# A2R-Lab/indy7-mpc

Measured on AMD Instinct MI355X. Metric: SQP-MPC solves/sec (Indy7 6-DOF, N=32), higher is better.
Workload: dtype f64

## Files before the change

### indy7_mpc_amd/csrc/i7m_admm.h

```cpp
#pragma once

#include "i7m_kernels.h"

namespace i7m {

struct AdmmCfg {
  double rho0, sigma, alpha, eps_abs, eps_rel, adapt_tol;
  int max_iter, check, scaling, gap, adapt_interval, pad;
};

struct AdmmArgs {
  SolveParams P;
  AdmmCfg A;
  const double* lin;
  const double* cost;
  const double* qpd;
  const double* xu;
  const double* xs;
  const int* active;
  double* sol;
  double *sx, *sz, *sy, *sq, *srho;
  double *Pq, *Pd, *I, *qs, *ls, *D, *E, *Dt, *Et, *R, *w;
  double* cs;
  int* iters;
  int* status;
  int sqp_iter;
  int b0;
  int ablate;
  const double* abase;
  long abytes;
};

constexpr int ADMM_FSTRIDE = 19;
constexpr int ADMM_SCALE_WPE = 2;
constexpr int ADMM_FACTOR_WPE = 2;
constexpr int ADM_REC = 300, REC_J = 180;
__device__ __forceinline__ int adm_lw(int i) { return i < 16 ? 2 * ((i + 2) / 2) : 18; }
__device__ __forceinline__ int adm_lrow(int i) {
  const int h = i >> 1;
  return i < 16 ? 2 * h * (h + 1) + (i & 1) * (2 * h + 2) : 144 + 18 * (i - 16);
}
__device__ __forceinline__ int adm_lrec(int i, int j) { return adm_lrow(i) + j; }
constexpr unsigned A5_OOB = 0x7ff00000u;
__device__ __forceinline__ __amdgpu_buffer_rsrc_t a4_rsrc(const void* base, long bytes) {
  const unsigned long long u = (unsigned long long)base;
  const unsigned lo = __builtin_amdgcn_readfirstlane((unsigned)u), hi = __builtin_amdgcn_readfirstlane((unsigned)(u >> 32));
  const int nb = __builtin_amdgcn_readfirstlane((int)bytes);
  return __builtin_amdgcn_make_buffer_rsrc((void*)(((unsigned long long)hi << 32) | lo), (short)0, nb, 0x00020000);
}
__device__ __forceinline__ void adm_stage_J(double* sJ, const double* Jc, int l) {
  for (int e = l; e < 216; e += 64) {
    const int i = e / 18, j = e - 18 * i;
    double v;
    if (i < 6) v = j == i ? Jc[i] : (j == 6 + i ? Jc[6 + i] : 0.0);
    else v = Jc[12 + 18 * (i - 6) + j];
    sJ[e] = v;
  }
}

// ... 112 lines not shown
    xPx += xe * px;
    qx += qe * xe;
  }
  pr = adm_max<W>(pr); zn = adm_max<W>(zn); an = adm_max<W>(an); pri = adm_max<W>(pri); pn = adm_max<W>(pn);
  dr = adm_max<W>(dr); qn = adm_max<W>(qn); atn = adm_max<W>(atn); pxn = adm_max<W>(pxn);
  dua = adm_max<W>(dua); dn = adm_max<W>(dn);
  xPx = adm_sum<W>(xPx); qx = adm_sum<W>(qx); sc = adm_sum<W>(sc);
  const double cinv = 1.0 / c;
  {
    const double p = pri / (pn + 1e-30), d = dua / (dn + 1e-30);
    double rn = rho * sqrt(p / (d + 1e-30));
    *rho_est = fmin(fmax(rn, 1e-6), 1e6);
  }
  dr *= cinv;
  const double ea = es * a.A.eps_abs, er = es * a.A.eps_rel;
  if (!(pr < ea + er * fmax(zn, an))) return false;
  if (!(dr < ea + er * cinv * fmax(qn, fmax(atn, pxn)))) return false;
  if (a.A.gap) {
    xPx *= cinv; qx *= cinv; sc *= cinv;
    const double gp = xPx + qx + sc;
    if (!(fabs(gp) < ea + er * fmax(fabs(xPx), fmax(fabs(qx), fabs(sc))))) return false;
  }
  return true;
}

__device__ __forceinline__ double adm_pq(const double* w, int i, int j) { return w[6] * (w[i] * w[j]); }
template <int CT>
__device__ __forceinline__ double adm_scale(const AdmmArgs& a, int b, int N, int T, int m, const double* LIN,
                                            const double* CO, const double* QD, const double* X, double* qold,
                                            double* Pq, double* Pd, double* Jb, double* Ib, double* qs, double* ls,
                                            double* D, double* E, double* sD, double* sE, double* sDt, double* sRM, int l) {
  constexpr int RT = 2 * CT / 3;
  const double dt = a.P.dt;
  double qv[CT], etv[RT], dtv[CT <= 9 ? CT : 1];
#pragma unroll
  for (int t = 0; t < CT; ++t) {
    const int e = l + 64 * t;
    qv[t] = 0.0;
    if (e < T) {
      sD[e] = 1.0;
      qv[t] = qold[e];
    }
  }
#pragma unroll
  for (int t = 0; t < RT; ++t)
    if (l + 64 * t < m) sE[l + 64 * t] = 1.0;
  wave_sync_fence();
  double c = 1.0;
  auto pcol = [&](const double* Cp, int k, int j, double dj) {
    const double* w = Cp + COST_STRIDE * k;
    const int jq = j < 6 ? j : 0;
    double mq = 0.0;
#pragma unroll
    for (int i = 0; i < 6; ++i) mq = fmax(mq, fabs(adm_pq(w, i, jq)) * (sD[18 * k + i] * dj) * c);
    const double pd = j < 12 ? w[7] : w[8];
    return j < 6 ? mq : fabs(pd) * (dj * dj) * c;
  };
  constexpr bool REG = CT <= 9;
  const int ks = l >> 1, hs = l & 1;
  const bool sv = REG && ks < N - 1;
  double av[REG ? 3 : 1][REG ? 18 : 1];
  if constexpr (REG) {
    const double* L = LIN + LIN_STRIDE * (sv ? ks : 0);
#pragma unroll
    for (int r = 0; r < 3; ++r)
#pragma unroll
      for (int j = 0; j < 18; ++j) {
// ... 34 lines not shown
      for (int j = 0; j < 18; ++j) {
        const long long u = __double_as_longlong(cm[j]);
        const int lo = __builtin_amdgcn_update_dpp(0, (int)u, 0xB1, 0xf, 0xf, true);
        const int hi = __builtin_amdgcn_update_dpp(0, (int)(u >> 32), 0xB1, 0xf, 0xf, true);
        cm[j] = fmax(cm[j], __longlong_as_double(((long long)hi << 32) | (unsigned int)lo));
      }
      if (sv) {
#pragma unroll
        for (int j = 0; j < 9; ++j) sDt[18 * kq + 9 * hs + j] = hs ? cm[9 + j] : cm[j];
      }
      wave_sync_fence();
    }
    AS_STAMP(1);
#pragma unroll 3
    for (int t = 0; t < CT; ++t) {
      const int e = min(lp + 64 * t, T - 1), k = e / 18, j = e - 18 * k;
      const double dj = sD[e];
      double mx = pcol(Cp, k, j, dj);
      const double ei = sE[12 * k + (j < 12 ? j : 0)] * dj;
      if (j < 12) mx = fmax(mx, ei);
      const int kk = k < N - 1 ? k : N - 2;
      const double* L = Lp + LIN_STRIDE * kk;
      const double* Eb = sE + 12 * (kk + 1);
      const int jb = j < 6 ? j : (j < 12 ? 30 + j : 60 + j);
      const double eid = Eb[j < 6 ? j : (j < 12 ? j - 6 : 0)] * (j < 6 ? 1.0 : dt) * dj;
      double mj = j < 12 ? eid : 0.0;
      if constexpr (REG) {
        mj = fmax(mj, sDt[e]);
      } else {
#pragma unroll
        for (int r = 0; r < 6; ++r) mj = fmax(mj, Eb[6 + r] * fabs(L[jb + 6 * r]) * dj);
      }
      if (k < N - 1) mx = fmax(mx, mj);
      if constexpr (REG) dtv[t] = 1.0 / sqrt(adm_limit(mx));
      else sDt[lp + 64 * t] = 1.0 / sqrt(adm_limit(mx));
    }
    AS_STAMP(2);
#pragma unroll
    for (int t = 0; t < RT; ++t) {
      const int r = min(lp + 64 * t, m - 1), blk = r / 12, i = r - 12 * blk;
      const double er = sE[r];
      double mx = er * sD[18 * blk + i];
      const int kk = blk > 0 ? blk - 1 : 0;
      const double* Db = sD + 18 * kk;
      const int i6 = i < 6 ? i : i - 6;
      const double mi = fmax(er * 1.0 * Db[i6], er * dt * Db[6 + i6]);
      double ml = 0.0;
      if constexpr (REG) {
        ml = sRM[r];
      } else {
        const double* L = Lp + LIN_STRIDE * kk;
#pragma unroll
        for (int j = 0; j < 18; ++j) {
          const int jb = j < 6 ? j : (j < 12 ? 30 + j : 60 + j);
          ml = fmax(ml, er * fabs(L[jb + 6 * i6]) * Db[j]);
        }
      }
      const double mj = i < 6 ? mi : ml;
      if (blk > 0) mx = fmax(mx, mj);
      etv[t] = 1.0 / sqrt(adm_limit(mx));
    }
    AS_STAMP(3);
    wave_sync_fence();
#pragma unroll
    for (int t = 0; t < CT; ++t) {
      const int e = lp + 64 * t;
      double dtt;
      if constexpr (CT <= 9) dtt = dtv[t];
      else dtt = sDt[e];
      if (e < T) sD[e] = sD[e] * dtt;
      qv[t] = dtt * qv[t];
    }
#pragma unroll
    for (int t = 0; t < RT; ++t)
      if (lp + 64 * t < m) sE[lp + 64 * t] = sE[lp + 64 * t] * etv[t];
    wave_sync_fence();
    AS_STAMP(4);
    double sm = 0.0, qm = 0.0;
#pragma unroll
    for (int t = 0; t < CT; ++t) {
      const int e = lp + 64 * t, ec = min(e, T - 1), k = ec / 18, j = ec - 18 * k;
      const double mx = pcol(Cp, k, j, sD[ec]);
      if (e < T) {
        sm += mx;
        qm = fmax(qm, fabs(qv[t]));
      }
    }
    sm = adm_wave_sum(sm);
    qm = adm_limit(adm_wave_max(qm));
    const double ct = 1.0 / adm_limit(fmax(sm / T, qm));
#pragma unroll
    for (int t = 0; t < CT; ++t) qv[t] = qv[t] * ct;
    c = c * ct;
    AS_STAMP(5);
  }
#undef AS_STAMP
#ifdef I7M_DIAG
  if (ss_on && l == 0) tl_write_stamps(ss_t, 6, a.ablate, 3);
#endif
  for (int e = l; e < T; e += 64) D[e] = sD[e];
  for (int r = l; r < m; r += 64) E[r] = sE[r];
#pragma unroll 4
// ... 175 lines not shown
        sL[18 * i + l] = v;
        if (l < adm_lw(i)) Rb[ADM_REC * k + adm_lrec(i, l)] = v;
      }
    }
    wave_sync();
    AF_STAMP(5);
    if (k < N - 1) {
#pragma unroll
      for (int t = 0; t < 4; ++t) {
        const int e = l + 64 * t;
        if (e < 216) {
          const int i = e / 18, j = e - 18 * i;
          const double acc = adm_dot2<18>(0.0, sJ + 18 * i, 1, sL + 18 * j, 1);
          const double cv = re * G[186 + i] * acc;
          sCp[FS * i + j] = cv;
        }
      }
    }
    wave_sync_fence();
    AF_STAMP(6);
  }
#undef AF_STAMP
#ifdef I7M_DIAG
  if (fs_on && l0 == 0) tl_write_stamps(fs_t, 7, a.ablate, 2);
#endif
}

template <int PH, int CT>
__device__ __forceinline__ void admm_body(const AdmmArgs& a) {
  const int b = a.b0 + blockIdx.x;
  const SolveParams& P = a.P;
  if (b >= P.B || (a.active && !a.active[b])) return;
  const int l = threadIdx.x, N = P.N, T = P.T, m = 12 * N;
  constexpr bool FAC = (PH & 8) != 0;
  __shared__ double sB[(PH & 1) ? 64 * CT : 756], sS[FAC ? 18 * ADMM_FSTRIDE : 1], sCp[FAC ? 12 * ADMM_FSTRIDE : 1];
  __shared__ double sD[(PH & 1) ? 64 * CT : 1], sE[(PH & 1) ? 64 * (2 * CT / 3) : 1], sRM[(PH & 1) ? 64 * (2 * CT / 3) : 1],
      sCO[(PH & 1) ? (64 * CT / 18 + 1) * COST_STRIDE : 1], sStg[FAC ? 2 * AF_STG : 1];
  double* sL = sB;
  double* sJ = sB + 540;
  const double* LIN = a.lin + (long)b * (N - 1) * LIN_STRIDE;
  const double* CO = a.cost + (long)b * N * COST_STRIDE;
  const double* QD = a.qpd + (long)b * (N - 1) * QPD_STRIDE;
  const double* X = a.xu + (long)b * T;
  double* qold = a.sq + (long)b * T;
  double* Pq = a.Pq + (long)b * N * 36;
  double* Pd = a.Pd + (long)b * T;
  double* Rb = a.R + (long)b * N * ADM_REC;
  double* Jb = Rb + REC_J;
  double* Ib = a.I + (long)b * m;
  double* qs = a.qs + (long)b * T;
  double* ls = a.ls + (long)b * m;
  double* D = a.D + (long)b * T;
  double* E = a.E + (long)b * m;
  if constexpr (PH & 1) {
    for (int e = l; e < N * COST_STRIDE; e += 64) sCO[e] = CO[e];
    const double c = adm_scale<CT>(a, b, N, T, m, LIN, sCO, QD, X, qold, Pq, Pd, Jb, Ib, qs, ls, D, E, sD, sE, sB, sRM, l);
    if (l == 0) a.cs[b] = c;
  }
  if constexpr (PH & 8) {
    adm_factor(a, N, a.srho[b], Pq, Pd, Ib, Rb, sS, sJ, sL, sCp, sStg, l);
  }
}

template <int CT>
__global__ void __launch_bounds__(64) __attribute__((amdgpu_waves_per_eu(ADMM_SCALE_WPE, ADMM_SCALE_WPE)))
k_admm_scale(AdmmArgs a) {
  admm_body<1, CT>(a);
}
__global__ void __launch_bounds__(64) __attribute__((amdgpu_waves_per_eu(ADMM_FACTOR_WPE, ADMM_FACTOR_WPE)))
k_admm_factor(AdmmArgs a) {
  admm_body<8, 1>(a);
}

}
```

### indy7_mpc_amd/csrc/i7m_admm_prep_tu.hip

```cpp
#include <hip/hip_runtime.h>
#include <hip/hip_ext.h>

#include <algorithm>
#include <cmath>

#include "../../include/indy7_mpc.h"

namespace {
#include "i7m_admm.h"
}

#ifdef I7M_DIAG
extern "C" int i7m_admm_prep_tu_set_timeline(void* p) { return i7m::tl_set(p); }
#endif

hipError_t i7m_launch_admm_prep(int kernel, int grid, hipStream_t s, hipEvent_t ea, hipEvent_t eb, const void* args) {
  const i7m::AdmmArgs& a = *static_cast<const i7m::AdmmArgs*>(args);
  if (kernel == 0)
    hipExtLaunchKernelGGL(i7m::k_admm_scale<9>, dim3(grid), dim3(64), 0, s, ea, eb, 0, a);
  else if (kernel == 1)
    hipExtLaunchKernelGGL(i7m::k_admm_scale<18>, dim3(grid), dim3(64), 0, s, ea, eb, 0, a);
  else if (kernel == 2)
    hipExtLaunchKernelGGL(i7m::k_admm_factor, dim3(grid), dim3(64), 0, s, ea, eb, 0, a);
  else
    return hipErrorInvalidValue;
  return hipGetLastError();
}
```

### indy7_mpc_amd/csrc/i7m_api.hip

```cpp
#include <hip/hip_runtime.h>
#include <hip/hip_ext.h>

#include <algorithm>
#include <atomic>
#include <cmath>
#include <cstdio>
#include <cstdlib>
#include <cstring>
#include <string>
#include <thread>
#include <vector>

#include "../../include/indy7_mpc.h"
#include "i7m_kernels.h"
#include "i7m_linearize.h"
#include "i7m_riccati_mfma.h"
#include "i7m_box.h"
#include "i7m_admm_iter.h"
#include "i7m_mpc.h"
#include "i7m_mpc_sampled.h"
#include "i7m_ctrl.h"
#include "i7m_plan.h"

#ifndef I7M_SRC_HASH
// ... 404 lines not shown
                            sol, goals, W.fext, active, st, alpha_out, iter, mode, W.lin, W.cost, second);
    });
  }
  return timed(h, s, I7M_K_LINESEARCH, [&](hipEvent_t ea, hipEvent_t eb) {
    hipExtLaunchKernelGGL(ls_kernel(h->spec, fw, nw), dim3(P.B), dim3(64 * nw), lds, s, ea, eb, 0, h->d_model, P, xu, xu_out,
                          sol, goals, W.fext, active, st, alpha_out, iter, mode, ln, cs, LsSplit{});
  });
}

BoxParams box_params(const i7m_handle* h) {
  BoxParams BP;
  BP.mask = h->cfg.box_mask;
  BP.max_iters = h->cfg.box_max_iters;
  BP.tol = h->cfg.box_tol;
  BP.theta = 0.2;
  BP.eta = 0.99;
  BP.z0 = 0.1;
  return BP;
}

struct StaggerMark {
  hipEvent_t ev;
  int at;
  bool recorded;
};
int record_mark(StaggerMark* m, int at, hipStream_t s) {
  if (!m || m->recorded || m->at != at) return I7M_OK;
  HIPCHK(hipEventRecord(m->ev, s));
  m->recorded = true;
  return I7M_OK;
}

int solve_qp(i7m_handle* h, hipStream_t s, const Bufs& W, const SolveParams& P, const double* xu, const double* xs,
             const int* active, double* sol, const double** out, int sqp_iter = 0, StaggerMark* mark = nullptr) {
  int rc;
  if (h->cfg.qp_mode == I7M_QP_ADMM) {
    *out = sol;
    if (P.B == 0) return I7M_OK;
    AdmmArgs a = W.adm;
    a.P = P;
    a.A = admm_cfg_of(h->cfg);
    a.lin = W.lin;
    a.cost = W.cost;
    a.qpd = W.qpd;
    a.xu = xu;
    a.xs = xs;
    a.active = active;
    a.sol = sol;
    a.sqp_iter = sqp_iter;
#ifdef I7M_DIAG
    a.ablate = h->ablate;
#endif
    a.b0 = 0;
    const int n = P.B;
    hipError_t e = hipSuccess;
    rc = timed(h, s, I7M_K_ADMM_PREP, [&](hipEvent_t ea, hipEvent_t eb) {
      if (admm_prep_ilp(h->tune, n)) {
        e = i7m_launch_admm_prep(P.N <= 32 ? 0 : 1, n, s, ea, nullptr, &a);
        if (e == hipSuccess) e = i7m_launch_admm_prep(2, n, s, nullptr, eb, &a);
        return;
      }
      if (P.N <= 32)
        hipExtLaunchKernelGGL(k_admm_scale<9>, dim3(n), dim3(64), 0, s, ea, nullptr, 0, a);
      else
        hipExtLaunchKernelGGL(k_admm_scale<18>, dim3(n), dim3(64), 0, s, ea, nullptr, 0, a);
      hipExtLaunchKernelGGL(k_admm_factor, dim3(n), dim3(64), 0, s, nullptr, eb, 0, a);
    });
    if (rc) return rc;
    if (e != hipSuccess) return fail(I7M_EHIP, std::string("k_admm_scale / k_admm_factor launch: ") + hipGetErrorString(e));
    if ((rc = record_mark(mark, 1, s))) return rc;
    rc = timed(h, s, I7M_K_ADMM, [&](hipEvent_t ea, hipEvent_t eb) {
      const dim3 g((n + 3) / 4);
      switch (admm_iter_kernel(h->tune, P.N, a.A.adapt_interval != 0, n)) {
        case AdmmIter::adapt: hipExtLaunchKernelGGL(k_admm_iter<true>, g, dim3(64), 0, s, ea, eb, 0, a); break;
        case AdmmIter::res: hipExtLaunchKernelGGL(k_admm_iter_res, dim3(n), dim3(64), 0, s, ea, eb, 0, a); break;
        case AdmmIter::iter2:
          hipExtLaunchKernelGGL(k_admm_iter2, dim3((n + 1) / 2), dim3(64), 0, s, ea, eb, 0, a);
          break;
        case AdmmIter::iter4: hipExtLaunchKernelGGL(k_admm_iter<false>, g, dim3(64), 0, s, ea, eb, 0, a); break;
      }
    });
    if (rc) return rc;
    return record_mark(mark, 2, s);
  }
  if ((rc = launch_riccati(h, s, W, P, xu, xs, active, sol))) return rc;
  *out = sol;
  if (h->cfg.qp_mode != I7M_QP_BOX || P.B == 0) return I7M_OK;
  const BoxParams BP = box_params(h);
  const dim3 g(P.B), blk(64);
  if (h->tune.ipm_mode != 2) {
    IpmFusedArgs fa{h->d_model, P, BP, xu, xs, W.lin, W.cost, W.qpd, active, W.kbuf, sol, sol,
                    W.bx, W.bzl, W.bzu, W.bsig, W.bh, W.bdxa, W.bst, W.bact, W.bhinv, W.bdh};
#ifdef I7M_DIAG
    fa.ablate = h->ablate;
#endif
    rc = timed(h, s, I7M_K_IPM_FUSED, [&](hipEvent_t ea, hipEvent_t eb) {
      if (h->tune.ipm_mode == 0)
        hipExtLaunchKernelGGL(k_ipm_fused<true>, g, blk, 0, s, ea, eb, 0, fa);
      else
        hipExtLaunchKernelGGL(k_ipm_fused<false>, g, blk, 0, s, ea, eb, 0, fa);
    });
    if (rc) return rc;
// ... 23 lines not shown
      if (rc) return rc;
    }
  }
  *out = W.bx;
  return I7M_OK;
}

int launch_fused(i7m_handle* h, hipStream_t s, const Bufs& W, const SolveParams& P, const double* xu_in, double* xu_out,
                 const double* xs, const double* goals, ProblemStats* st) {
  const int nw = fused_waves(h->tune, P.B);
  const int launches = h->tune.pipeline == I7M_PIPE_FUSED_ITER ? h->cfg.max_sqp_iters : 1;
  for (int i = 0; i < launches; ++i) {
    hipError_t e = hipSuccess;
    const int rc = timed(h, s, I7M_K_SQP_FUSED, [&](hipEvent_t ea, hipEvent_t eb) {
      e = i7m_launch_sqp_fused(h->spec, nw, h->fext_frame == I7M_WRENCH_WORLD, launches > 1 ? i : -1, s, ea, eb, h->d_model,
                               &P, i == 0 ? xu_in : xu_out, xu_out, xs, goals, W.fext, W.lin, W.cost, W.qpd, W.kbuf,
                               W.sol, W.active, st);
    });
    if (rc) return rc;
    if (e != hipSuccess) return fail(I7M_EHIP, std::string("k_sqp_fused launch: ") + hipGetErrorString(e));
  }
  return I7M_OK;
}

int run_sqp(i7m_handle* h, int B, const double* d_xu_in, double* d_xu, const double* d_xs, const double* d_goals,
            int goal_stride, ProblemStats* d_st, long b0 = 0, hipStream_t s = nullptr, StaggerMark* mark = nullptr) {
  const Bufs W = bufs_at(h, b0);
  const SolveParams P = params_of(h, B, goal_stride);
  if (!s) s = h->stream;
  if (!d_st) d_st = W.stats;
  int* act = W.active;
  double* qbuf = W.sol;
  if (use_fused(h->tune, h->cfg.qp_mode)) return launch_fused(h, s, W, P, d_xu_in, d_xu, d_xs, d_goals, d_st);
  if (h->cfg.qp_mode == I7M_QP_ADMM && B > 0) {
    HIPCHK(hipMemsetAsync(W.adm.iters, 0xff, (size_t)B * I7M_MAX_SQP * sizeof(int), s));
    HIPCHK(hipMemsetAsync(W.adm.status, 0xff, (size_t)B * I7M_MAX_SQP * sizeof(int), s));
  }
  for (int it = 0; it < h->cfg.max_sqp_iters; ++it) {
    const double* xin = it == 0 ? d_xu_in : d_xu;
    int rc;
    if (it == 0)
      rc = launch_linearize(h, s, W, P, xin, d_goals, nullptr, act, d_st);
    else
      rc = launch_linearize(h, s, W, P, xin, d_goals, act);
    if (rc) return rc;
    const double* qsol = nullptr;
    if ((rc = solve_qp(h, s, W, P, xin, d_xs, act, qbuf, &qsol, it, mark))) return rc;
    if ((rc = launch_linesearch(h, s, W, P, xin, d_xu, qsol, d_goals, act, d_st, nullptr, it,
                                h->cfg.qp_mode == I7M_QP_ADMM ? 2 : 0, true)))
      return rc;
  }
  return I7M_OK;
}

void drop_graphs(i7m_handle* h) {
  for (auto& g : h->graphs) (void)hipGraphExecDestroy(g.exec);
  h->graphs.clear();
}

int run_sqp_graphed(i7m_handle* h, int B, const double* d_xu_in, double* d_xu, const double* d_xs, const double* d_goals,
                    int goal_stride, ProblemStats* d_st) {
  if (!h->tune.use_graph || h->timing)
    return run_sqp(h, B, d_xu_in, d_xu, d_xs, d_goals, goal_stride, d_st);
  const int hf = h->has_fext ? 1 : 0;
  i7m_handle::GraphEntry* hit = nullptr;
  for (auto& g : h->graphs)
    if (g.B == B && g.goal_stride == goal_stride && g.has_fext == hf && g.xu_in == d_xu_in && g.xu == d_xu && g.xs == d_xs &&
        g.goals == d_goals && g.st == d_st && g.stream == (const void*)h->stream)
      hit = &g;
  if (!hit) {
    HIPCHK(hipStreamBeginCapture(h->stream, hipStreamCaptureModeThreadLocal));
    const int rc = run_sqp(h, B, d_xu_in, d_xu, d_xs, d_goals, goal_stride, d_st);
    hipGraph_t graph = nullptr;
    const hipError_t e = hipStreamEndCapture(h->stream, &graph);
    if (rc) {
      if (graph) (void)hipGraphDestroy(graph);
      return rc;
    }
    if (e != hipSuccess) return fail(I7M_EHIP, std::string("hipStreamEndCapture: ") + hipGetErrorString(e));
    hipGraphExec_t exec = nullptr;
// ... 179 lines not shown
  for (int r = 0; r < 2; ++r) {
    const long lo = cuts[r], hi = cuts[r + 1];
    HIPCHK(hipStreamWaitEvent(h->cs[r], h->ev_order, 0));
    if (hi <= lo) continue;
    if (r == 1 && mark.recorded) HIPCHK(hipStreamWaitEvent(h->cs[1], mark.ev, 0));
    const int rc = body(lo, (int)(hi - lo), h->cs[r], r == 0 ? &mark : nullptr);
    if (rc) {
      const std::string msg = g_err;
      for (int q = 0; q <= r; ++q) {
        (void)hipEventRecord(h->ev_done[q], h->cs[q]);
        (void)hipStreamWaitEvent(h->stream, h->ev_done[q], 0);
      }
      g_err = msg;
      return rc;
    }
  }
  for (int r = 0; r < 2; ++r) {
    HIPCHK(hipEventRecord(h->ev_done[r], h->cs[r]));
    HIPCHK(hipStreamWaitEvent(h->stream, h->ev_done[r], 0));
  }
  return I7M_OK;
}

int admm_rows(i7m_handle* h, int B, AdmmArgs* a) {
  if (!h) return fail(I7M_EINVAL, "null handle");
  if (h->cfg.qp_mode != I7M_QP_ADMM) return fail(I7M_EINVAL, "handle is not in I7M_QP_ADMM mode");
  if (B < 0 || B > h->cfg.max_batch) return fail(I7M_EINVAL, "batch outside [0, max_batch]");
  if (B == 0) return I7M_OK;
  HIPCHK(hipSetDevice(h->dev));
  *a = admm_layout(h, 0);
  return I7M_OK;
}

int admm_reset_rows(i7m_handle* h, long lo, long n, int what, hipStream_t s, const double* rho, hipMemcpyKind kind) {
  const size_t T = h->T, m = 12 * (size_t)h->N;
  const AdmmArgs a = admm_layout(h, lo);
  if (what & I7M_ADMM_RESET_PRIMAL) {
    HIPCHK(hipMemsetAsync(a.sx, 0, n * T * 8, s));
    HIPCHK(hipMemsetAsync(a.sz, 0, n * m * 8, s));
    HIPCHK(hipMemsetAsync(a.sq, 0, n * T * 8, s));
  }
  if (what & I7M_ADMM_RESET_DUAL) HIPCHK(hipMemsetAsync(a.sy, 0, n * m * 8, s));
  if (what & I7M_ADMM_RESET_RHO) HIPCHK(hipMemcpyAsync(a.srho, rho, (size_t)n * 8, kind, s));
  return I7M_OK;
}

struct Workspace : Carved {
  i7m_handle* h;
  template <size_t NB>
  Workspace(i7m_handle* hh, const size_t (&bytes)[NB]) : h(hh) {
    alloc(bytes, (int)NB, false);
  }
  Workspace(const Workspace&) = delete;
  ~Workspace() {
    (void)hipStreamSynchronize(h->stream);
    release();
  }
};

struct LoopStart {
  size_t rows;
  std::vector<double> goals;
  std::vector<int> ones;
  LoopStart(const i7m_handle* h, size_t rows_, size_t instances, const double* endpoints)
      : rows(rows_), goals(rows_ * 3 * h->N), ones(instances, 1) {
    for (size_t k = 0; k < goals.size(); ++k) goals[k] = endpoints[k % 3];
  }
  LoopStart(const i7m_handle* h, size_t rows_, size_t instances, int H, const double* ref, long L, int ref_stride,
            const int32_t* ref_phase)
      : rows(rows_), goals(rows_ * 3 * h->N), ones(instances, 1) {
    const size_t W = 3 * h->N;
    for (size_t b = 0; b < rows; ++b)
      for (size_t e = 0; e < W; ++e)
        goals[b * W + e] = ref[track_index(ref_phase ? ref_phase[b / H] : 0, 0, (long)(e / 3), L) * ref_stride + e % 3];
  }
};
// ... 276 lines not shown
  if (!h) return;
  (void)hipSetDevice(h->dev);
  if (h->stream) (void)hipStreamSynchronize(h->stream);
  for (void* p : h->owned) (void)hipFree(p);
  ctrl_release(h);
  for (auto& t : h->ev) {
    (void)hipEventDestroy(t.a);
    (void)hipEventDestroy(t.b);
  }
  for (auto e : h->pool) (void)hipEventDestroy(e);
  for (auto e : h->ev_in) (void)hipEventDestroy(e);
  for (auto e : h->ev_cmp) (void)hipEventDestroy(e);
  drop_graphs(h);
  if (h->cs2) {
    (void)hipStreamSynchronize(h->cs2);
    (void)hipStreamDestroy(h->cs2);
  }
  for (int c = 0; c < 2; ++c) {
    if (h->cs[c]) {
      (void)hipStreamSynchronize(h->cs[c]);
      (void)hipStreamDestroy(h->cs[c]);
    }
    if (h->ev_done[c]) (void)hipEventDestroy(h->ev_done[c]);
  }
  if (h->ev_order) (void)hipEventDestroy(h->ev_order);
  if (h->ev_rmark) (void)hipEventDestroy(h->ev_rmark);
  if (h->own) (void)hipStreamDestroy(h->own);
  delete h;
}

int i7m_set_stream(i7m_handle* h, void* stream) {
  if (!h) return fail(I7M_EINVAL, "null handle");
  if (h->ctrl.open) return session_open();
  h->stream = stream ? (hipStream_t)stream : h->own;
  return I7M_OK;
}

int i7m_set_external_wrench(i7m_handle* h, int32_t B, const double* fext, int32_t frame) {
  if (!h) return fail(I7M_EINVAL, "null handle");
  if (h->ctrl.open) return session_open();
  if (!fext) {
    h->has_fext = false;
    drop_graphs(h);
    return I7M_OK;
  }
  if (frame != I7M_WRENCH_LOCAL && frame != I7M_WRENCH_WORLD)
    return fail(I7M_EINVAL, "frame must be I7M_WRENCH_LOCAL or I7M_WRENCH_WORLD");
  if (B < 1 || B > h->cfg.max_batch) return fail(I7M_EINVAL, "external wrench batch outside [1, max_batch]");
  HIPCHK(hipSetDevice(h->dev));
  return install_wrench(h, B, fext, frame);
}

int i7m_reset(i7m_handle* h) {
  if (!h) return fail(I7M_EINVAL, "null handle");
  if (h->ctrl.open) return session_open();
  HIPCHK(hipSetDevice(h->dev));
  HIPCHK(hipStreamSynchronize(h->stream));
  drop_graphs(h);
  if (h->cfg.qp_mode == I7M_QP_ADMM) {
    const int rc = i7m_admm_reset(h, h->cfg.max_batch, I7M_ADMM_RESET_ALL);
    if (rc) return rc;
  }
  return i7m_reset_kernel_times(h);
}

int i7m_admm_reset(i7m_handle* h, int32_t B, int32_t what) {
  if (h && h->ctrl.open) return session_open();
  AdmmArgs a{};
  int rc = admm_rows(h, B, &a);
  if (rc) return rc;
  if (what & ~I7M_ADMM_RESET_ALL) return fail(I7M_EINVAL, "unknown I7M_ADMM_RESET_* bits");
  if (B == 0) return I7M_OK;
  const std::vector<double> rho((size_t)B, h->cfg.admm_rho);
  if ((rc = admm_reset_rows(h, 0, B, what, h->stream, rho.data(), hipMemcpyHostToDevice))) return rc;
  HIPCHK(hipMemsetAsync(a.iters, 0xff, (size_t)B * I7M_MAX_SQP * sizeof(int), h->stream));
  HIPCHK(hipMemsetAsync(a.status, 0xff, (size_t)B * I7M_MAX_SQP * sizeof(int), h->stream));
  return i7m_synchronize(h);
}

int i7m_get_admm_stats(i7m_handle* h, int32_t B, int32_t* iters, double* rho) {
  AdmmArgs a{};
  const int rc = admm_rows(h, B, &a);
  if (rc || B == 0) return rc;
  if (iters) HIPCHK(hipMemcpyAsync(iters, a.iters, (size_t)B * I7M_MAX_SQP * sizeof(int), hipMemcpyDeviceToHost, h->stream));
  if (rho) HIPCHK(hipMemcpyAsync(rho, a.srho, (size_t)B * 8, hipMemcpyDeviceToHost, h->stream));
  return i7m_synchronize(h);
}

int i7m_get_admm_status(i7m_handle* h, int32_t B, int32_t* status) {
  if (!h || !status) return fail(I7M_EINVAL, "null handle or output");
  AdmmArgs a{};
  const int rc = admm_rows(h, B, &a);
  if (rc || B == 0) return rc;
  HIPCHK(hipMemcpyAsync(status, a.status, (size_t)B * I7M_MAX_SQP * sizeof(int), hipMemcpyDeviceToHost, h->stream));
  return i7m_synchronize(h);
}

int i7m_get_admm_dual(i7m_handle* h, int32_t B, double* y) {
  if (!h || !y) return fail(I7M_EINVAL, "null handle or output");
  AdmmArgs a{};
  int rc = admm_rows(h, B, &a);
  if (rc || B == 0) return rc;
  const long m = 12 * h->N;
  std::vector<double> e((size_t)B * m), c((size_t)B);
  if ((rc = copy_out(h, y, a.sy, (size_t)B * m)) || (rc = copy_out(h, e.data(), a.E, (size_t)B * m)) ||
      (rc = copy_out(h, c.data(), a.cs, (size_t)B)))
    return rc;
  HIPCHK(hipStreamSynchronize(h->stream));
  for (long b = 0; b < B; ++b)
    for (long r = 0; r < m; ++r) y[b * m + r] = e[b * m + r] * y[b * m + r] / c[b];
// ... 275 lines not shown
  const GoalSource& gs = c.goal;
  const bool track = c.kind == SampledKind::tracking;
  if (G == 0) return I7M_OK;
  HIPCHK(hipSetDevice(h->dev));
  const int N = (int)h->N, B = G * H;
  const size_t T = h->T;
  const bool admm = h->cfg.qp_mode == I7M_QP_ADMM;
  size_t bytes[TRACKING_WS_COUNT];
  tracking_ws_bytes(G, H, N, num_steps, gs.n_endpoints, o.n_actual, noise != nullptr, gs.L, gs.ref_stride,
                    gs.ref_phase != nullptr, bytes);
  const GroupStart start(h, G, H, c.xstart, gs);
  Workspace ws(h, bytes);
  if (!ws.base) return fail(I7M_ENOMEM, who + ": device allocation failed");
  double *d_ep = ws.at<double>(SWS_EP), *d_xcur = ws.at<double>(SWS_XCUR), *d_xub = ws.at<double>(SWS_XUB),
         *d_fact = ws.at<double>(SWS_FACT), *d_noise = bytes[SWS_NOISE] ? ws.at<double>(SWS_NOISE) : nullptr,
         *d_dist = ws.at<double>(SWS_DIST), *d_q = ws.at<double>(SWS_Q), *d_fb = ws.at<double>(SWS_FB),
         *d_rho0 = ws.at<double>(SWS_RHO0), *d_ref = track ? ws.at<double>(TWS_REF) : nullptr,
         *d_ee = track ? ws.at<double>(TWS_EE) : nullptr;
  int *d_best = ws.at<int>(SWS_BEST), *d_gi = ws.at<int>(SWS_GI), *d_alive = ws.at<int>(SWS_ALIVE),
      *d_bh = ws.at<int>(SWS_BH), *d_phase = bytes[TWS_PHASE] ? ws.at<int>(TWS_PHASE) : nullptr;
  const size_t hist = history_rows(num_steps, G);
  if ((rc = stage_start(h, start, gs, G, d_rho0, d_ref, d_phase))) return rc;
  if ((rc = loop_instances(h, start.rows, gs.endpoints, gs.n_endpoints, d_ep, d_gi, d_alive))) return rc;
  if ((rc = copy_in(h, d_xcur, c.xstart, (size_t)G * 12))) return rc;
  if ((rc = copy_in(h, d_fact, c.f_actual, 6 * (size_t)o.n_actual * G))) return rc;
  if (d_noise && (rc = copy_in(h, d_noise, noise, 3 * (size_t)num_steps * B))) return rc;
  HIPCHK(hipMemsetAsync(d_best, 0, 4 * (size_t)G, h->stream));
  if ((rc = install_wrench(h, B, c.fhyp, o.frame))) return rc;
  rc = run_ranges(h, B, [&](long lo, int n, hipStream_t s, StaggerMark* mark) -> int {
    const long glo = lo / H;
    const int ng = n / H;
    double *xu = h->d_xu + lo * T, *out = h->d_out + lo * T, *xs = h->d_xs + lo * 12, *g = h->d_goal + lo * 3 * N;
    auto reset = [&](int what) {
      return admm && what ? admm_reset_rows(h, lo, n, what, s, d_rho0 + lo, hipMemcpyDeviceToDevice) : I7M_OK;
    };
    SampledArgs a{};
    a.N = N;
    a.H = H;
    a.n_endpoints = gs.n_endpoints;
    a.frame_world = o.frame == I7M_WRENCH_WORLD;
    a.keep_best = o.keep_best != 0;
    a.sim_dt = o.sim_dt;
    a.decay = o.decay;
    a.xs = xs;
    a.XU = xu;
    a.xu_new = out;
    a.goals = g;
    a.fext = h->d_fext + lo * 6;
    a.xcur = d_xcur + glo * 12;
    a.xub = d_xub + glo * T;
    a.best = d_best + glo;
    a.goal_idx = d_gi + glo;
    a.alive = d_alive + glo;
    a.endpoints = track ? nullptr : d_ep;
    a.ref = d_ref;
    a.ref_phase = d_phase ? d_phase + glo : nullptr;
    a.L = (int)gs.L;
    a.ref_stride = gs.ref_stride;
    int rc3;
    if ((rc3 = reset(I7M_ADMM_RESET_ALL))) return rc3;
    if ((rc3 = run_sqp(h, n, xu, out, xs, g, 3, nullptr, lo, s, mark))) return rc3;
    for (int i = 0; i <= num_steps; ++i) {
      a.select = i == 0 ? 2 : 1;
      a.plant = i < num_steps;
      const size_t rec = ((size_t)std::max(i - 1, 0)) * G + glo, cur = (size_t)std::min(i, std::max(num_steps - 1, 0)) * G + glo;
      a.noise = d_noise && i > 0 ? d_noise + ((size_t)(i - 1) * B + lo) * 3 : nullptr;
      a.best_out = d_bh + rec;
// ... 32 lines not shown
int i7m_mpc_run_sampled(i7m_handle* h, int32_t G, int32_t H, const double* xstart, const double* endpoints,
                        int32_t n_endpoints, int32_t num_steps, const double* fhyp, const double* f_actual,
                        const double* noise, const i7m_sampled_opts* opts, double* dist_out, int32_t* best_out,
                        double* q_out, double* fbest_out, double* xcur_out, double* xu_best_out, double* fhyp_out) {
  if (!h) return fail(I7M_EINVAL, "null handle");
  const SampledCall c = describe_call(h, SampledKind::endpoints, G, H, num_steps, opts,
                                      GoalSource::of_endpoints(endpoints, n_endpoints), xstart, fhyp, f_actual, dist_out);
  return sampled_loop(h, "mpc_run_sampled", c, noise, dist_out, best_out, q_out, nullptr, fbest_out, xcur_out,
                      xu_best_out, fhyp_out);
}

int i7m_mpc_run_tracking(i7m_handle* h, int32_t G, int32_t H, const double* xstart, const double* ref, int32_t L,
                         int32_t ref_stride, const int32_t* ref_phase, const int32_t* ref_offset, int32_t num_steps,
                         const double* fhyp, const double* f_actual, const double* noise, const i7m_sampled_opts* opts,
                         double* err_out, int32_t* best_out, double* q_out, double* ee_out, double* fbest_out,
                         double* xcur_out, double* xu_best_out, double* fhyp_out) {
  if (!h) return fail(I7M_EINVAL, "null handle");
  const SampledCall c = describe_call(h, SampledKind::tracking, G, H, num_steps, opts,
                                      GoalSource::of_reference(ref, L, ref_stride, ref_phase, ref_offset), xstart, fhyp,
                                      f_actual, err_out);
  return sampled_loop(h, "mpc_run_tracking", c, noise, err_out, best_out, q_out, ee_out, fbest_out, xcur_out,
                      xu_best_out, fhyp_out);
}

}

namespace {

int ctrl_solve(i7m_handle* h, int what) {
  const CtrlSession& c = h->ctrl;
  const int B = c.G * c.H;
  int rc;
  if (h->cfg.qp_mode == I7M_QP_ADMM && what &&
      (rc = admm_reset_rows(h, 0, B, what, h->stream, c.dev.at<double>(CWS_RHO0), hipMemcpyDeviceToDevice)))
    return rc;
  return run_sqp(h, B, h->d_xu, h->d_out, h->d_xs, h->d_goal, 3, nullptr);
}

void ctrl_launch_select(i7m_handle* h, const CtrlArgs& a) {
  hipLaunchKernelGGL(k_ctrl_select, dim3(h->ctrl.G), dim3((h->ctrl.H + 63) / 64 * 64), 0, h->stream, a);
}

}

extern "C" {

int i7m_ctrl_begin(i7m_handle* h, int32_t G, int32_t H, const double* x0, const double* ref, int32_t L,
                   int32_t ref_stride, const int32_t* ref_phase, const double* fhyp, const i7m_sampled_opts* opts,
                   double* u_out) {
  const std::string who = "ctrl_begin";
  if (!h) return fail(I7M_EINVAL, "null handle");
  if (h->ctrl.open) return fail(I7M_EINVAL, who + ": a controller session is already open on this handle");
  const SampledCall call = describe_call(h, SampledKind::session, G, H, 0, opts,
                                         GoalSource::of_reference(ref, L, ref_stride, ref_phase, nullptr), x0, fhyp, nullptr,
                                         nullptr);
  int rc;
  if ((rc = check_call(who, call))) return rc;
  const i7m_sampled_opts& o = call.o;
  HIPCHK(hipSetDevice(h->dev));
  HIPCHK(hipStreamSynchronize(h->stream));
  const int N = (int)h->N;
  CtrlSession& c = h->ctrl;
  size_t db[CTRL_WS_COUNT], hb[CTRL_HS_COUNT];
  ctrl_ws_bytes(G, H, N, L, ref_stride, ref_phase != nullptr, db);
  ctrl_host_bytes(G, H, hb);
  if (!c.dev.alloc(db, CTRL_WS_COUNT, false)) {
    ctrl_release(h);
// ... 163 lines not shown
```

### indy7_mpc_amd/csrc/i7m_plan.h

```cpp
#pragma once

#include <algorithm>
#include <cmath>
#include <cstdlib>
#include <cstring>
#include <string>

#include "../../include/indy7_mpc.h"

#if defined(__HIPCC__)
#define I7M_PLAN_HD __host__ __device__
#else
#define I7M_PLAN_HD
#endif

namespace i7m {

struct Tuning {
  int ls_waves = 0;
  int ls_tail = 0;
  bool use_graph = false;
  int ric_w2 = -1;
  int ric_bc = -1;
  int h2h_chunks = 0;
  int h2h_pipe = 2;
  int h2h_taper = 1;
  int admm_stagger = 1;
  int admm_stagger_min_b = 3072;
  int admm_iter2 = -1;
  int admm_res = -1;
  int admm_res_max = 256;
  int admm_prep_ilp = -1;
  int admm_prep_ilp_max = 1024;
  int ipm_mode = 1;
  int pipeline = I7M_PIPE_AUTO;
  bool generic = false;
};

constexpr int RIC_W2_MAX_B = 128;
constexpr int RIC_PRIO_MIN_B = 768;
constexpr int LS_W4_MAX_B = 768, FUSED_W4_MAX_B = 256;
constexpr int ADMM_ITER2_MAX_B = 512;
constexpr int ADMM_RES_MAX_N = 32;
constexpr int H2H_3_MIN_B = 3072, H2H_2_MIN_B = 2048;

inline bool tuning_from_env(const i7m_config& cfg, Tuning* t, std::string* err) {
  for (const char* name : {"I7M_ADMM_CHUNK", "I7M_DEV_RANGES", "I7M_ADMM_CHAINS", "I7M_ADMM_RANGES", "I7M_ADMM_SPLIT",
                           "I7M_STAGGER_MODES", "I7M_ADMM_ITER_DYN_LDS"})
    if (std::getenv(name)) {
      *err = std::string(name) + " is set, but this A/B knob was retired (it measured slower; DESIGN.md has the "
                                 "numbers): unset it";
      return false;
    }
  *t = Tuning{};
  if (const char* e = std::getenv("I7M_IPM"))
    t->ipm_mode = std::strcmp(e, "split") == 0 ? 2 : (std::strcmp(e, "delta") == 0 ? 0 : 1);
  if (const char* e = std::getenv("I7M_LS_TAIL")) t->ls_tail = std::min(std::max(std::atoi(e), 0), 3);
  if (const char* e = std::getenv("I7M_LS_WAVES")) t->ls_waves = std::atoi(e) == 4 ? 4 : (std::atoi(e) == 2 ? 2 : 1);
  if (const char* e = std::getenv("I7M_GRAPH")) t->use_graph = std::atoi(e) != 0;
  if (const char* e = std::getenv("I7M_RIC_W2")) t->ric_w2 = std::atoi(e) != 0;
  if (const char* e = std::getenv("I7M_RIC_BC")) {
    const int v = std::atoi(e) & 7;
    t->ric_bc = (v == 4 || v == 5) ? (v & 3) : v;
  }
  t->h2h_chunks = cfg.h2h_chunks;
  if (const char* e = std::getenv("I7M_H2H_CHUNKS")) t->h2h_chunks = std::atoi(e);
  if (const char* e = std::getenv("I7M_H2H_PIPE")) t->h2h_pipe = std::min(std::max(std::atoi(e), 0), 3);
  if (const char* e = std::getenv("I7M_H2H_TAPER")) t->h2h_taper = std::atoi(e) != 0;
  if (const char* e = std::getenv("I7M_ADMM_STAGGER")) {
    t->admm_stagger = std::min(std::max(std::atoi(e), 0), 4);
    if (t->admm_stagger > 2) {
      *err = std::string("I7M_ADMM_STAGGER=") + e + ": the stagger marks 3 and 4 were retired (they measured "
                                                    "slower; DESIGN.md §4.7): use 0, 1 or 2";
      return false;
    }
  }
  if (const char* e = std::getenv("I7M_ADMM_STAGGER_MIN_B")) t->admm_stagger_min_b = std::max(std::atoi(e), 2);
  if (const char* e = std::getenv("I7M_ADMM_ITER2")) t->admm_iter2 = std::min(std::max(std::atoi(e), -1), 1);
  if (const char* e = std::getenv("I7M_ADMM_RES")) t->admm_res = std::min(std::max(std::atoi(e), -1), 1);
  if (const char* e = std::getenv("I7M_ADMM_RES_MAX")) t->admm_res_max = std::max(std::atoi(e), 0);
  if (const char* e = std::getenv("I7M_ADMM_PREP_ILP")) t->admm_prep_ilp = std::min(std::max(std::atoi(e), -1), 1);
  if (const char* e = std::getenv("I7M_ADMM_PREP_ILP_MAX")) t->admm_prep_ilp_max = std::max(std::atoi(e), 0);
  if (t->h2h_chunks < 0 || t->h2h_chunks > 64) {
    *err = "h2h_chunks must be in [0, 64]";
    return false;
  }
  t->pipeline = cfg.pipeline;
  if (const char* e = std::getenv("I7M_PIPE"))
    t->pipeline = std::strcmp(e, "fused") == 0 ? I7M_PIPE_FUSED
                  : std::strcmp(e, "fused_iter") == 0 ? I7M_PIPE_FUSED_ITER
                  : std::strcmp(e, "split") == 0 ? I7M_PIPE_SPLIT
                  : t->pipeline;
  if (const char* e = std::getenv("I7M_GENERIC")) t->generic = std::atoi(e) != 0;
  return true;
}

enum class Ablate { known, retired, unknown };
struct AblateStatus {
  Ablate kind;
  const char* msg;
};
inline AblateStatus ablate_status(int v) {
  if (v == 0 || v == 21 || (v >= 40 && v <= 44) || v >= 100000) return {Ablate::known, nullptr};
  for (int r : {1, 2, 4, 6, 8, 10, 11, 13, 18, 19})
    if (v == r)
      return {Ablate::retired, "I7M_ABLATE names a Riccati / line-search timing variant that was retired (DESIGN.md "
                               "§7 has its numbers; commit a2cf0e7 is the last tree that builds it): unset it"};
  return {Ablate::unknown, "I7M_ABLATE is set to a value that no kernel acts on: unset it"};
}


enum class AdmmIter { adapt, res, iter2, iter4 };
inline AdmmIter admm_iter_kernel(const Tuning& t, int N, bool adaptive_rho, int n) {
  if (adaptive_rho) return AdmmIter::adapt;
  if (N <= ADMM_RES_MAX_N && (t.admm_res > 0 || (t.admm_res < 0 && n <= t.admm_res_max))) return AdmmIter::res;
  if (t.admm_iter2 > 0 || (t.admm_iter2 < 0 && n <= ADMM_ITER2_MAX_B)) return AdmmIter::iter2;
  return AdmmIter::iter4;
}

inline bool admm_prep_ilp(const Tuning& t, int n) {
  return t.admm_prep_ilp > 0 || (t.admm_prep_ilp < 0 && n <= t.admm_prep_ilp_max);
}

struct RicVariant {
  bool w2;
  int bc;
};
inline RicVariant riccati_variant(const Tuning& t, int B, bool vout) {
  const int bc = t.ric_bc >= 0 ? t.ric_bc : 3 | (B >= RIC_PRIO_MIN_B ? 4 : 0);
  const bool w2 = !vout && (t.ric_w2 >= 0 ? t.ric_w2 != 0 : B <= RIC_W2_MAX_B);
  return {w2, bc};
}

inline int ls_waves(const Tuning& t, int B) { return t.ls_waves > 0 ? t.ls_waves : (B <= LS_W4_MAX_B ? 4 : 1); }
inline int fused_waves(const Tuning& t, int B) { return t.ls_waves > 0 ? t.ls_waves : (B <= FUSED_W4_MAX_B ? 4 : 1); }

inline bool use_fused(const Tuning& t, int qp_mode) {
  return qp_mode == I7M_QP_DIRECT && (t.pipeline == I7M_PIPE_FUSED || t.pipeline == I7M_PIPE_FUSED_ITER);
}

inline bool stagger_applies(const Tuning& t, int qp_mode, int B) {
  return qp_mode == I7M_QP_ADMM && t.admm_stagger > 0 && B >= t.admm_stagger_min_b;
}
inline long stagger_cut(int B) { return std::min<long>(((long)(B / 2) + 3) / 4 * 4, B); }
inline long stagger_cut_grouped(int B, int H) {
  const long L = std::max(H, 4);
  return std::min<long>(((long)B + 2 * L - 1) / (2 * L) * L, B);
}

inline int h2h_chunks_for(const Tuning& t, int qp_mode, int B) {
  int n;
  if (t.h2h_chunks > 0) n = t.h2h_chunks;
  else if (stagger_applies(t, qp_mode, B)) n = 2;
  else n = B >= H2H_3_MIN_B ? 3 : (B >= H2H_2_MIN_B ? 2 : 1);
// ... 194 lines not shown
```

Measured before the change: 393,000.

## Fuse ADMM scale and factor kernels and fold record resets into kernels

Adds a fused k_admm_prep kernel that runs scaling and factorization in one launch, with a single overlaid shared-memory buffer sized to the larger phase. It is enabled by default (fused_min=0), which removes one kernel launch and a launch gap per SQP iteration. The two per-solve hipMemsetAsync calls for the iteration and status records are replaced by writes inside the prep kernel on the first SQP iteration. The reset path now uses one custom kernel instead of several memsets and a memcpy. The scale phase also drops its register array for the dt scales and always goes through shared memory, which could add some LDS traffic.

Result: faster. 397,600, median of 6 (+1.2%).

```diff
diff --git a/indy7_mpc_amd/csrc/i7m_admm.h b/indy7_mpc_amd/csrc/i7m_admm.h
--- a/indy7_mpc_amd/csrc/i7m_admm.h
+++ b/indy7_mpc_amd/csrc/i7m_admm.h
@@ -25,6 +25,7 @@
   int* iters;
   int* status;
   int sqp_iter;
+  int init_rec;
   int b0;
   int ablate;
   const double* abase;
@@ -203,7 +204,7 @@
                                             double* D, double* E, double* sD, double* sE, double* sDt, double* sRM, int l) {
   constexpr int RT = 2 * CT / 3;
   const double dt = a.P.dt;
-  double qv[CT], etv[RT], dtv[CT <= 9 ? CT : 1];
+  double qv[CT], etv[RT];
 #pragma unroll
   for (int t = 0; t < CT; ++t) {
     const int e = l + 64 * t;
@@ -304,8 +305,7 @@
         for (int r = 0; r < 6; ++r) mj = fmax(mj, Eb[6 + r] * fabs(L[jb + 6 * r]) * dj);
       }
       if (k < N - 1) mx = fmax(mx, mj);
-      if constexpr (REG) dtv[t] = 1.0 / sqrt(adm_limit(mx));
-      else sDt[lp + 64 * t] = 1.0 / sqrt(adm_limit(mx));
+      sDt[lp + 64 * t] = 1.0 / sqrt(adm_limit(mx));
     }
     AS_STAMP(2);
 #pragma unroll
@@ -337,9 +337,7 @@
 #pragma unroll
     for (int t = 0; t < CT; ++t) {
       const int e = lp + 64 * t;
-      double dtt;
-      if constexpr (CT <= 9) dtt = dtv[t];
-      else dtt = sDt[e];
+      const double dtt = sDt[e];
       if (e < T) sD[e] = sD[e] * dtt;
       qv[t] = dtt * qv[t];
     }
@@ -581,12 +579,14 @@
   const SolveParams& P = a.P;
   if (b >= P.B || (a.active && !a.active[b])) return;
   const int l = threadIdx.x, N = P.N, T = P.T, m = 12 * N;
-  constexpr bool FAC = (PH & 8) != 0;
-  __shared__ double sB[(PH & 1) ? 64 * CT : 756], sS[FAC ? 18 * ADMM_FSTRIDE : 1], sCp[FAC ? 12 * ADMM_FSTRIDE : 1];
-  __shared__ double sD[(PH & 1) ? 64 * CT : 1], sE[(PH & 1) ? 64 * (2 * CT / 3) : 1], sRM[(PH & 1) ? 64 * (2 * CT / 3) : 1],
-      sCO[(PH & 1) ? (64 * CT / 18 + 1) * COST_STRIDE : 1], sStg[FAC ? 2 * AF_STG : 1];
-  double* sL = sB;
-  double* sJ = sB + 540;
+  constexpr bool SC = (PH & 1) != 0, FAC = (PH & 8) != 0;
+  constexpr int FS = ADMM_FSTRIDE, RT = 2 * CT / 3;
+  constexpr int oD = 64 * CT, oE = oD + 64 * CT, oRM = oE + 64 * RT, oCO = oRM + (CT <= 9 ? 64 * RT : 0);
+  constexpr int nSC = SC ? oCO + (64 * CT / 18 + 1) * COST_STRIDE : 0;
+  constexpr int oS = 756, oCp = oS + 18 * FS, oStg = oCp + 12 * FS;
+  constexpr int nFA = FAC ? oStg + 2 * AF_STG : 0;
+  static_assert(oStg % 2 == 0, "the stage DMA writes 16-byte pieces");
+  __shared__ __attribute__((aligned(16))) double sM[nSC > nFA ? nSC : nFA];
   const double* LIN = a.lin + (long)b * (N - 1) * LIN_STRIDE;
   const double* CO = a.cost + (long)b * N * COST_STRIDE;
   const double* QD = a.qpd + (long)b * (N - 1) * QPD_STRIDE;
@@ -601,13 +601,24 @@
   double* ls = a.ls + (long)b * m;
   double* D = a.D + (long)b * T;
   double* E = a.E + (long)b * m;
-  if constexpr (PH & 1) {
+  if constexpr (SC) {
+    if (a.init_rec && l < I7M_MAX_SQP) {
+      a.iters[(long)b * I7M_MAX_SQP + l] = -1;
+      a.status[(long)b * I7M_MAX_SQP + l] = -1;
+    }
+    double* sCO = sM + oCO;
     for (int e = l; e < N * COST_STRIDE; e += 64) sCO[e] = CO[e];
-    const double c = adm_scale<CT>(a, b, N, T, m, LIN, sCO, QD, X, qold, Pq, Pd, Jb, Ib, qs, ls, D, E, sD, sE, sB, sRM, l);
+    const double c = adm_scale<CT>(a, b, N, T, m, LIN, sCO, QD, X, qold, Pq, Pd, Jb, Ib, qs, ls, D, E, sM + oD, sM + oE, sM,
+                                   sM + oRM, l);
     if (l == 0) a.cs[b] = c;
   }
-  if constexpr (PH & 8) {
-    adm_factor(a, N, a.srho[b], Pq, Pd, Ib, Rb, sS, sJ, sL, sCp, sStg, l);
+  if constexpr (SC && FAC) {
+    asm volatile("s_waitcnt vmcnt(0) lgkmcnt(0)" ::: "memory");
+    __builtin_amdgcn_fence(__ATOMIC_RELEASE, "workgroup");
+    __builtin_amdgcn_fence(__ATOMIC_ACQUIRE, "workgroup");
+  }
+  if constexpr (FAC) {
+    adm_factor(a, N, a.srho[b], Pq, Pd, Ib, Rb, sM + oS, sM + 540, sM, sM + oCp, sM + oStg, l);
   }
 }
 
@@ -620,5 +631,36 @@
 k_admm_factor(AdmmArgs a) {
   admm_body<8, 1>(a);
 }
-
-}
+template <int CT>
+__global__ void __launch_bounds__(64) __attribute__((amdgpu_waves_per_eu(ADMM_SCALE_WPE, ADMM_SCALE_WPE)))
+k_admm_prep(AdmmArgs a) {
+  admm_body<9, CT>(a);
+}
+
+struct AdmmResetArgs {
+  double *sx, *sz, *sy, *sq, *srho;
+  int *iters, *status;
+  const double* rho_src;
+  double rho0;
+  long n;
+  int T, m, what, records;
+};
+__global__ void __launch_bounds__(256) k_admm_reset(AdmmResetArgs r) {
+  const long nT = r.n * r.T, nm = r.n * r.m, nr = r.n * I7M_MAX_SQP;
+  const long step = (long)gridDim.x * blockDim.x;
+  for (long i = (long)blockIdx.x * blockDim.x + threadIdx.x; i < nT; i += step) {
+    if (r.what & I7M_ADMM_RESET_PRIMAL) {
+      r.sx[i] = 0.0;
+      r.sq[i] = 0.0;
+      if (i < nm) r.sz[i] = 0.0;
+    }
+    if ((r.what & I7M_ADMM_RESET_DUAL) && i < nm) r.sy[i] = 0.0;
+    if ((r.what & I7M_ADMM_RESET_RHO) && i < r.n) r.srho[i] = r.rho_src ? r.rho_src[i] : r.rho0;
+    if (r.records && i < nr) {
+      r.iters[i] = -1;
+      r.status[i] = -1;
+    }
+  }
+}
+
+}
diff --git a/indy7_mpc_amd/csrc/i7m_admm_prep_tu.hip b/indy7_mpc_amd/csrc/i7m_admm_prep_tu.hip
--- a/indy7_mpc_amd/csrc/i7m_admm_prep_tu.hip
+++ b/indy7_mpc_amd/csrc/i7m_admm_prep_tu.hip
@@ -22,6 +22,10 @@
     hipExtLaunchKernelGGL(i7m::k_admm_scale<18>, dim3(grid), dim3(64), 0, s, ea, eb, 0, a);
   else if (kernel == 2)
     hipExtLaunchKernelGGL(i7m::k_admm_factor, dim3(grid), dim3(64), 0, s, ea, eb, 0, a);
+  else if (kernel == 3)
+    hipExtLaunchKernelGGL(i7m::k_admm_prep<9>, dim3(grid), dim3(64), 0, s, ea, eb, 0, a);
+  else if (kernel == 4)
+    hipExtLaunchKernelGGL(i7m::k_admm_prep<18>, dim3(grid), dim3(64), 0, s, ea, eb, 0, a);
   else
     return hipErrorInvalidValue;
   return hipGetLastError();
diff --git a/indy7_mpc_amd/csrc/i7m_api.hip b/indy7_mpc_amd/csrc/i7m_api.hip
--- a/indy7_mpc_amd/csrc/i7m_api.hip
+++ b/indy7_mpc_amd/csrc/i7m_api.hip
@@ -460,7 +460,8 @@
 }
 
 int solve_qp(i7m_handle* h, hipStream_t s, const Bufs& W, const SolveParams& P, const double* xu, const double* xs,
-             const int* active, double* sol, const double** out, int sqp_iter = 0, StaggerMark* mark = nullptr) {
+             const int* active, double* sol, const double** out, int sqp_iter = 0, StaggerMark* mark = nullptr,
+             bool init_records = false) {
   int rc;
   if (h->cfg.qp_mode == I7M_QP_ADMM) {
     *out = sol;
@@ -476,6 +477,7 @@
     a.active = active;
     a.sol = sol;
     a.sqp_iter = sqp_iter;
+    a.init_rec = init_records;
 #ifdef I7M_DIAG
     a.ablate = h->ablate;
 #endif
@@ -483,19 +485,27 @@
     const int n = P.B;
     hipError_t e = hipSuccess;
     rc = timed(h, s, I7M_K_ADMM_PREP, [&](hipEvent_t ea, hipEvent_t eb) {
-      if (admm_prep_ilp(h->tune, n)) {
-        e = i7m_launch_admm_prep(P.N <= 32 ? 0 : 1, n, s, ea, nullptr, &a);
+      const bool ilp = admm_prep_ilp(h->tune, n), wide = P.N > 32;
+      if (admm_prep_fused(h->tune, n)) {
+        if (ilp)
+          e = i7m_launch_admm_prep(wide ? 4 : 3, n, s, ea, eb, &a);
+        else if (wide)
+          hipExtLaunchKernelGGL(k_admm_prep<18>, dim3(n), dim3(64), 0, s, ea, eb, 0, a);
+        else
+          hipExtLaunchKernelGGL(k_admm_prep<9>, dim3(n), dim3(64), 0, s, ea, eb, 0, a);
+      } else if (ilp) {
+        e = i7m_launch_admm_prep(wide ? 1 : 0, n, s, ea, nullptr, &a);
         if (e == hipSuccess) e = i7m_launch_admm_prep(2, n, s, nullptr, eb, &a);
-        return;
+      } else {
+        if (wide)
+          hipExtLaunchKernelGGL(k_admm_scale<18>, dim3(n), dim3(64), 0, s, ea, nullptr, 0, a);
+        else
+          hipExtLaunchKernelGGL(k_admm_scale<9>, dim3(n), dim3(64), 0, s, ea, nullptr, 0, a);
+        hipExtLaunchKernelGGL(k_admm_factor, dim3(n), dim3(64), 0, s, nullptr, eb, 0, a);
       }
-      if (P.N <= 32)
-        hipExtLaunchKernelGGL(k_admm_scale<9>, dim3(n), dim3(64), 0, s, ea, nullptr, 0, a);
-      else
-        hipExtLaunchKernelGGL(k_admm_scale<18>, dim3(n), dim3(64), 0, s, ea, nullptr, 0, a);
-      hipExtLaunchKernelGGL(k_admm_factor, dim3(n), dim3(64), 0, s, nullptr, eb, 0, a);
     });
+    if (e != hipSuccess) return fail(I7M_EHIP, std::string("ADMM preparation launch: ") + hipGetErrorString(e));
     if (rc) return rc;
-    if (e != hipSuccess) return fail(I7M_EHIP, std::string("k_admm_scale / k_admm_factor launch: ") + hipGetErrorString(e));
     if ((rc = record_mark(mark, 1, s))) return rc;
     rc = timed(h, s, I7M_K_ADMM, [&](hipEvent_t ea, hipEvent_t eb) {
       const dim3 g((n + 3) / 4);
@@ -585,10 +595,6 @@
   int* act = W.active;
   double* qbuf = W.sol;
   if (use_fused(h->tune, h->cfg.qp_mode)) return launch_fused(h, s, W, P, d_xu_in, d_xu, d_xs, d_goals, d_st);
-  if (h->cfg.qp_mode == I7M_QP_ADMM && B > 0) {
-    HIPCHK(hipMemsetAsync(W.adm.iters, 0xff, (size_t)B * I7M_MAX_SQP * sizeof(int), s));
-    HIPCHK(hipMemsetAsync(W.adm.status, 0xff, (size_t)B * I7M_MAX_SQP * sizeof(int), s));
-  }
   for (int it = 0; it < h->cfg.max_sqp_iters; ++it) {
     const double* xin = it == 0 ? d_xu_in : d_xu;
     int rc;
@@ -598,7 +604,7 @@
       rc = launch_linearize(h, s, W, P, xin, d_goals, act);
     if (rc) return rc;
     const double* qsol = nullptr;
-    if ((rc = solve_qp(h, s, W, P, xin, d_xs, act, qbuf, &qsol, it, mark))) return rc;
+    if ((rc = solve_qp(h, s, W, P, xin, d_xs, act, qbuf, &qsol, it, mark, it == 0))) return rc;
     if ((rc = launch_linesearch(h, s, W, P, xin, d_xu, qsol, d_goals, act, d_st, nullptr, it,
                                 h->cfg.qp_mode == I7M_QP_ADMM ? 2 : 0, true)))
       return rc;
@@ -844,16 +850,15 @@
   return I7M_OK;
 }
 
-int admm_reset_rows(i7m_handle* h, long lo, long n, int what, hipStream_t s, const double* rho, hipMemcpyKind kind) {
-  const size_t T = h->T, m = 12 * (size_t)h->N;
+int admm_reset_rows(i7m_handle* h, long lo, long n, int what, hipStream_t s, const double* rho, bool records = false) {
+  if (n <= 0 || (!what && !records)) return I7M_OK;
   const AdmmArgs a = admm_layout(h, lo);
-  if (what & I7M_ADMM_RESET_PRIMAL) {
-    HIPCHK(hipMemsetAsync(a.sx, 0, n * T * 8, s));
-    HIPCHK(hipMemsetAsync(a.sz, 0, n * m * 8, s));
-    HIPCHK(hipMemsetAsync(a.sq, 0, n * T * 8, s));
-  }
-  if (what & I7M_ADMM_RESET_DUAL) HIPCHK(hipMemsetAsync(a.sy, 0, n * m * 8, s));
-  if (what & I7M_ADMM_RESET_RHO) HIPCHK(hipMemcpyAsync(a.srho, rho, (size_t)n * 8, kind, s));
+  const AdmmResetArgs r{a.sx, a.sz, a.sy, a.sq, a.srho, a.iters, a.status, rho, h->cfg.admm_rho, n,
+                        (int)h->T, 12 * (int)h->N, what, records ? 1 : 0};
+  const long work = (what & (I7M_ADMM_RESET_PRIMAL | I7M_ADMM_RESET_DUAL)) ? n * h->T : n * I7M_MAX_SQP;
+  const int grid = (int)std::min<long>((work + 255) / 256, 4096);
+  hipLaunchKernelGGL(k_admm_reset, dim3(grid), dim3(256), 0, s, r);
+  HIPCHK(hipGetLastError());
   return I7M_OK;
 }
 
@@ -1196,7 +1201,12 @@
 int i7m_set_stream(i7m_handle* h, void* stream) {
   if (!h) return fail(I7M_EINVAL, "null handle");
   if (h->ctrl.open) return session_open();
-  h->stream = stream ? (hipStream_t)stream : h->own;
+  hipStream_t next = stream ? (hipStream_t)stream : h->own;
+  if (next != h->stream && h->stream == h->own) {
+    HIPCHK(hipSetDevice(h->dev));
+    HIPCHK(hipStreamSynchronize(h->stream));
+  }
+  h->stream = next;
   return I7M_OK;
 }
 
@@ -1235,11 +1245,7 @@
   if (rc) return rc;
   if (what & ~I7M_ADMM_RESET_ALL) return fail(I7M_EINVAL, "unknown I7M_ADMM_RESET_* bits");
   if (B == 0) return I7M_OK;
-  const std::vector<double> rho((size_t)B, h->cfg.admm_rho);
-  if ((rc = admm_reset_rows(h, 0, B, what, h->stream, rho.data(), hipMemcpyHostToDevice))) return rc;
-  HIPCHK(hipMemsetAsync(a.iters, 0xff, (size_t)B * I7M_MAX_SQP * sizeof(int), h->stream));
-  HIPCHK(hipMemsetAsync(a.status, 0xff, (size_t)B * I7M_MAX_SQP * sizeof(int), h->stream));
-  return i7m_synchronize(h);
+  return admm_reset_rows(h, 0, B, what, h->stream, nullptr, true);
 }
 
 int i7m_get_admm_stats(i7m_handle* h, int32_t B, int32_t* iters, double* rho) {
@@ -1581,7 +1587,7 @@
     const int ng = n / H;
     double *xu = h->d_xu + lo * T, *out = h->d_out + lo * T, *xs = h->d_xs + lo * 12, *g = h->d_goal + lo * 3 * N;
     auto reset = [&](int what) {
-      return admm && what ? admm_reset_rows(h, lo, n, what, s, d_rho0 + lo, hipMemcpyDeviceToDevice) : I7M_OK;
+      return admm && what ? admm_reset_rows(h, lo, n, what, s, d_rho0 + lo) : I7M_OK;
     };
     SampledArgs a{};
     a.N = N;
@@ -1680,7 +1686,7 @@
   const int B = c.G * c.H;
   int rc;
   if (h->cfg.qp_mode == I7M_QP_ADMM && what &&
-      (rc = admm_reset_rows(h, 0, B, what, h->stream, c.dev.at<double>(CWS_RHO0), hipMemcpyDeviceToDevice)))
+      (rc = admm_reset_rows(h, 0, B, what, h->stream, c.dev.at<double>(CWS_RHO0))))
     return rc;
   return run_sqp(h, B, h->d_xu, h->d_out, h->d_xs, h->d_goal, 3, nullptr);
 }
diff --git a/indy7_mpc_amd/csrc/i7m_plan.h b/indy7_mpc_amd/csrc/i7m_plan.h
--- a/indy7_mpc_amd/csrc/i7m_plan.h
+++ b/indy7_mpc_amd/csrc/i7m_plan.h
@@ -32,6 +32,8 @@
   int admm_res_max = 256;
   int admm_prep_ilp = -1;
   int admm_prep_ilp_max = 1024;
+  int admm_prep_fused = -1;
+  int admm_prep_fused_min = 0;
   int ipm_mode = 1;
   int pipeline = I7M_PIPE_AUTO;
   bool generic = false;
@@ -81,6 +83,8 @@
   if (const char* e = std::getenv("I7M_ADMM_RES_MAX")) t->admm_res_max = std::max(std::atoi(e), 0);
   if (const char* e = std::getenv("I7M_ADMM_PREP_ILP")) t->admm_prep_ilp = std::min(std::max(std::atoi(e), -1), 1);
   if (const char* e = std::getenv("I7M_ADMM_PREP_ILP_MAX")) t->admm_prep_ilp_max = std::max(std::atoi(e), 0);
+  if (const char* e = std::getenv("I7M_ADMM_PREP_FUSED")) t->admm_prep_fused = std::min(std::max(std::atoi(e), -1), 1);
+  if (const char* e = std::getenv("I7M_ADMM_PREP_FUSED_MIN")) t->admm_prep_fused_min = std::max(std::atoi(e), 0);
   if (t->h2h_chunks < 0 || t->h2h_chunks > 64) {
     *err = "h2h_chunks must be in [0, 64]";
     return false;
@@ -120,6 +124,10 @@
 
 inline bool admm_prep_ilp(const Tuning& t, int n) {
   return t.admm_prep_ilp > 0 || (t.admm_prep_ilp < 0 && n <= t.admm_prep_ilp_max);
+}
+
+inline bool admm_prep_fused(const Tuning& t, int n) {
+  return t.admm_prep_fused > 0 || (t.admm_prep_fused < 0 && n >= t.admm_prep_fused_min);
 }
 
 struct RicVariant {
```
